# dblanm/gnn-manip

Measured on AMD Instinct MI355X. Metric: rollout steps/sec (N particles, 10 MP steps, hidden=128), higher is better.
Workload: dtype f32; 1 GPU; north_star target: N=100k dense synthetic scene, conn_r=0.015, max_neighbours=20, hidden=128, 10 MP steps; n_particles=100000, hidden=128, edges_last_step=1966056, k_steps=6, candidates_per_gpu=1, parallelism=candidate-parallel x1

## Files before the change

gnn_manip_amd/csrc/hedge.h:

```cpp
#pragma once
#include "common.h"
#include "mlp.h"

namespace gm {

struct EdgeBlockHeader {
    int n_blocks;
    int n_groups;
    int n_graphs;
    int n_per_graph;
    int n_stitch;
    int pad[3];
};
struct EdgeBlocks {
    EdgeBlockHeader* hdr;
    int* gblk;
    int2* blk;
    int2* seg;
    int* head;
    int* stitch;
    int* stitch_list;
    int64_t max_blocks;
};
size_t edge_blocks_ints(int64_t n_nodes, int64_t edge_capacity);
// ... 4 lines not shown

constexpr int kPackH3Max = 16;
struct PackH3Job {
    const float* W1;
    int W1_col0;
    int W1_ld;
    const float* W2;
    const float* W3;
    const float* b1;
    const float* b2;
    const float* b3;
    const float* gamma;
    const float* beta;
    float* dst;
    int enc_k1;
};
size_t h3_image_floats();
int pack_h3(const PackH3Job* jobs, int n, hipStream_t s);

int launch_edge_sys(const EdgeArgs& a, const EdgeBlocks& t, int64_t edge_capacity, hipStream_t s);
inline const float* edge_sys_p_scale(const float* h3_image) { return h3_image; }

struct NodeSysArgs {
    const float* h;
    const float* agg;
    const float* Q;
    float* h_out;
    const float* image;
    int n;
    int* flags;
// ... 5 lines not shown
struct ProjSysArgs {
    const float* h;
    float* P;
    float* Q;
    const float* img_p;
    const float* img_q;
    const float* scale_p;
    const float* scale_q;
    int n;
    int* flags;
    ProfState* prof;
    int precision;
};
int launch_proj_sys(const ProjSysArgs& a, hipStream_t s);
int launch_node_proj_sys(const NodeSysArgs& a, const ProjSysArgs& p, hipStream_t s);
int launch_agg_stitch(float* agg, const float* side, const EdgeBlocks& t, int64_t n, ProfState* prof, hipStream_t s);
constexpr int64_t kSysNodeMinNodes = 32 * 256 * 6;
int launch_edge_sys_enc(const EdgeArgs& a, hipStream_t s);
bool edge_sys_fits(int64_t n_nodes, int64_t edge_capacity);
constexpr int kEdgePadRows = 32;
int zero_edge_pad_rows(const CsrHeader* hdr, float* e, int row_floats, hipStream_t s);

}
```

gnn_manip_amd/csrc/hedge.hip:

```cpp
#include <type_traits>
#include "common.h"
#include "mlp.h"
#include "hedge.h"
#include "hmlp.h"
#include "hmma_dev.h"
#include "blocks_dev.h"

namespace gm {

namespace {

constexpr int H = 128;
constexpr int BE = 32;
constexpr int SYS_THREADS = 768;
static_assert(BE == kBlockEdges, "block tables and the systolic kernels agree on the block size");
#ifdef HEDGE_STAMPS
__device__ unsigned long long g_sys_stamps[3 * 32 * 8 + 32];
#define SYS_STAMP(tick, slot)                                                                                         \
    do {                                                                                                              \
        if (blockIdx.x == 0 && jb == 0 && lane0 == 0 && (tick) >= 16 && (tick) < 48) {                                \
            g_sys_stamps[(role * 32 + (tick) - 16) * 8 + (slot)] = __builtin_readcyclecounter();                     \
            if (role == 0 && (slot) == 0) g_sys_stamps[3 * 32 * 8 + (tick) - 16] = __builtin_amdgcn_s_memrealtime(); \
        }                                                                                                             \
    } while (0)
// ... 45 lines not shown
    return (g & 7) == 0 ? (i & 7) * (g >> 3) + (i >> 3) : i;
}

__device__ __forceinline__ int s_clamp0(int v, int hi) {
    int r;
    asm("s_max_i32 %0, %1, 0\n\ts_min_i32 %0, %0, %2" : "=s"(r) : "s"(v), "s"(hi) : "scc");
    return r;
}

extern __shared__ __attribute__((aligned(16))) char smem[];
#define LDS(T, off) (*reinterpret_cast<T*>(smem + (off)))
__device__ __forceinline__ unsigned opaque(unsigned v) { asm volatile("" : "+v"(v)); return v; }
__device__ __forceinline__ int tick_no(int t) { asm volatile("" : "+s"(t)); return t; }
#define GM_SB __builtin_amdgcn_sched_barrier(0)

template <int NP>
__device__ __forceinline__ void acc_to_image(const floatx16& a, char* smem, unsigned addr) {
#pragma unroll
    for (int q = 0; q < 2; ++q) {
        float v[8];
#pragma unroll
        for (int j = 0; j < 8; ++j) v[j] = relu(a[8 * q + j]);
        uintx2 h0, l0, h1, l1;
        if constexpr (NP == 3) {
            split4(v[0], v[1], v[2], v[3], h0, l0);
            split4(v[4], v[5], v[6], v[7], h1, l1);
        } else {
            hi4(v[0], v[1], v[2], v[3], h0);
            hi4(v[4], v[5], v[6], v[7], h1);
        }
        LDS(uintx4, addr + (q * 2 + 0) * 1024) = uintx4{h0[0], h0[1], h1[0], h1[1]};
        if constexpr (NP == 3) LDS(uintx4, addr + (q * 2 + 1) * 1024) = uintx4{l0[0], l0[1], l1[0], l1[1]};
    }
}

template <int NP, class F>
__device__ __forceinline__ void mlp_layer(floatx16& acc, const floatx16& c0, const half8 (&wh)[8], const half8 (&wl)[8], char* smem, unsigned a0, unsigned a1, F&& side) {
// ... 979 lines not shown
}

constexpr size_t NODE_PROJ_LDS_BYTES = NODE_LDS_BYTES > PROJ_LDS_BYTES ? NODE_LDS_BYTES : PROJ_LDS_BYTES;
static_assert(NODE_PROJ_LDS_BYTES <= 160 * 1024, "LDS budget");

template <int NP>
__global__ void __launch_bounds__(SYS_THREADS, 1) sys_node_proj_kernel(const float* a_h, float* a_h_out, const float* __restrict__ a_agg, float* a_Q, const float* __restrict__ a_hw,
                                                                            float* __restrict__ a_P, const float* __restrict__ a_wp, const float* __restrict__ a_wq,
                                                                            const float* __restrict__ a_sp, const float* __restrict__ a_sq, int a_n, int* a_flags,
                                                                            float a_eps) {
    sys_node_body<NP>(a_h, a_agg, a_Q, a_h_out, a_hw, a_n, a_flags, a_eps);
    __builtin_amdgcn_s_setprio(0);
    sys_proj_body<LD_SC1, NP>(a_h_out, a_P, a_Q, a_wp, a_wq, a_sp, a_sq, a_n, a_flags);
}

__global__ void __launch_bounds__(256) agg_stitch_kernel(float* __restrict__ agg, const float* __restrict__ side, const int* __restrict__ stitch,
                                                          const int* __restrict__ stitch_list, const int* __restrict__ head,
                                                          const EdgeBlockHeader* __restrict__ tab, int n) {
    const int ng = tab->n_groups, ns = tab->n_stitch;
    const int c = threadIdx.x & 7;
    for (int k = (blockIdx.x * 256 + threadIdx.x) >> 3; k < ns; k += (gridDim.x * 256) >> 3) {
        const int v = stitch_list[k];
        if (v < 0 || v >= n) continue;
        const int g0 = stitch[v];
        if (g0 < 0 || g0 >= ng || head[g0] != v) continue;
        floatx4 a[4];
#pragma unroll
        for (int q = 0; q < 4; ++q) a[q] = *reinterpret_cast<floatx4*>(agg + (size_t)v * H + 16 * c + 4 * q);
        int g = g0;
        do {
// ... 8 lines not shown

struct PackH3Jobs {
    int n;
    const float* W1[kPackH3Max];
    int c1[kPackH3Max];
    const float* W2[kPackH3Max];
    const float* W3[kPackH3Max];
    const float* b1[kPackH3Max];
    const float* b2[kPackH3Max];
    const float* b3[kPackH3Max];
    const float* gamma[kPackH3Max];
    const float* beta[kPackH3Max];
    float* dst[kPackH3Max];
    int enc_k1[kPackH3Max];
    int ld1[kPackH3Max];
};

constexpr int H3_PACK_THREADS = 1024;
__global__ void __launch_bounds__(H3_PACK_THREADS) pack_h3_kernel(PackH3Jobs J) {
    __shared__ float red[H3_PACK_THREADS];
    __shared__ float tsc[4];
    __shared__ float cmean[H + 1];
    const int job = blockIdx.x, tid = threadIdx.x;
    const float* Wl[3] = {J.W1[job], J.W2[job], J.W3[job]};
    if (tid < H) {
        float a = 0.f;
        for (int o = 0; o < H; ++o) a += J.W3[job][(size_t)o * H + tid];
        cmean[tid] = a * (1.0f / H);
    } else if (tid == H) {
        float a = 0.f;
        for (int o = 0; o < H; ++o) a += J.b3[job][o];
        cmean[H] = a * (1.0f / H);
    }
    __syncthreads();
    const int k1 = J.enc_k1[job];
    const bool enc = k1 > 0;
    const int ld[3] = {enc ? k1 : (J.ld1[job] > 0 ? J.ld1[job] : 3 * H), H, H}, c0[3] = {J.c1[job], 0, 0};
    const float* bl[3] = {J.b1[job], J.b2[job], J.b3[job]};
    float m_est = enc ? kHmRawInputRms : 1.f, U_prev = 1.f;
    if (tid == 0) tsc[3] = 0.f;
    __shared__ float capv;
    if (tid == 0) capv = 3.0e38f;
    for (int l = 0; l < 3; ++l) {
        float ss = 0.f, wm = 0.f;
        const int cols = l == 0 ? ld[0] : H;
        for (int i = tid; i < H * cols; i += H3_PACK_THREADS) {
            const int col = i % cols;
            float v = Wl[l][(size_t)(i / cols) * ld[l] + (l == 0 ? 0 : c0[l]) + col];
            if (l == 2) v -= cmean[col];
            ss = fmaf(v, v, ss);
            if (l != 0 || enc || (col >= c0[0] && col < c0[0] + H)) wm = fmaxf(wm, fabsf(v));
        }
        red[tid] = ss;
        __syncthreads();
        for (int s = H3_PACK_THREADS / 2; s > 0; s >>= 1) {
            if (tid < s) red[tid] += red[tid + s];
            __syncthreads();
        }
        const float ss_all = red[0];
        __syncthreads();
        red[tid] = wm;
        __syncthreads();
        for (int s = H3_PACK_THREADS / 2; s > 0; s >>= 1) {
            if (tid < s) red[tid] = fmaxf(red[tid], red[tid + s]);
            __syncthreads();
        }
        if (tid == 0) {
            const float wmax = red[0];
            float bs = 0.f, bmax = 0.f;
            for (int o = 0; o < H; ++o) {
                const float bv = bl[l][o] - (l == 2 ? cmean[H] : 0.f);
                bs = fmaf(bv, bv, bs);
                bmax = fmaxf(bmax, fabsf(bv));
            }
            const float g2 = ss_all / (float)H * 0.5f;
            float m = sqrtf(fmaf(enc ? 0.f : 0.5f, bs / (float)H, g2 * m_est * m_est));
            if (!(m > 1.0e-30f) || !(m < 1.0e30f)) m = 1.f;
            auto pow2 = [](float want, bool nearest) {
                if (!(want > 0.f) || !(want < 3.0e38f)) return 1.f;
                int ex;
                const float f = frexpf(want, &ex);
                int sh = (nearest && f >= 0.70710678f) ? ex : ex - 1;
                sh = sh < -100 ? -100 : (sh > 100 ? 100 : sh);
                return ldexpf(1.f, sh);
            };
            float t = pow2(kHmTargetRms / m, true) / U_prev;
            if (wmax > 0.f && wmax < 3.0e38f) {
                if (wmax * t > 8192.0f) t = pow2(8192.0f / wmax, false);
                if (wmax * t < 0.0625f) t = 2.f * pow2(0.0625f / wmax, false);
            }
            tsc[l] = t;
            tsc[3] = m;
            if (enc && bmax > 0.f) capv = fminf(capv, pow2(4096.0f / (U_prev * t * bmax), false));
        }
        __syncthreads();
        m_est = tsc[3];
        U_prev *= tsc[l];
        __syncthreads();
    }
    const float T1 = tsc[0], T2 = T1 * tsc[1], T3 = T2 * tsc[2];
    float* dst = J.dst[job];
    if (tid == 0) { dst[0] = T1; dst[1] = 1.0f / T3; dst[2] = capv; dst[3] = 0.f; }
    float* vec = dst + HW_HEADER_FLOATS;
    for (int i = tid; i < H; i += H3_PACK_THREADS) {
        vec[4 * H + i] = J.b1[job][i] * T1;
        vec[i] = J.b2[job][i] * T2;
        vec[H + i] = (J.b3[job][i] - cmean[H]) * T3;
        vec[2 * H + i] = J.gamma[job][i];
        vec[3 * H + i] = J.beta[job][i];
    }
    _Float16* img = reinterpret_cast<_Float16*>(dst + HW_HEADER_FLOATS + HW_VEC_FLOATS);
    for (int idx = tid; idx < 3 * 4 * 8 * 64 * 8; idx += H3_PACK_THREADS) {
        const int j = idx & 7, lane = (idx >> 3) & 63, ks = (idx >> 9) & 7, w = (idx >> 12) & 3, l = idx >> 14;
        const int i = lane & 31, kg = lane >> 5;
        const int kcol = 16 * ks + 8 * (j >> 2) + 4 * kg + (j & 3);
        const bool pad = l == 0 && enc && kcol >= k1;
        const float v = pad ? 0.f : (Wl[l][(size_t)(32 * w + i) * ld[l] + c0[l] + kcol] - (l == 2 ? cmean[kcol] : 0.f)) * tsc[l];
        const _Float16 h = (_Float16)v;
        const _Float16 lo = (_Float16)(v - (float)h);
        const size_t base = ((((size_t)(l * 4 + w) * 8 + ks) * 2) * 64 + lane) * 8 + j;
        img[base] = h;
        img[base + 64 * 8] = lo;
    }
}

__global__ void __launch_bounds__(256) edge_blocks_plan_kernel(const int* __restrict__ in_ptr, int n_nodes, const int* n_per_dev, int n_per_host,
                                                               EdgeBlockHeader* tab, int* gblk, int max_graphs) {
    if (threadIdx.x == 0) edge_blocks_plan(in_ptr, n_nodes, n_per_dev, n_per_host, tab, gblk, max_graphs);
}

__global__ void __launch_bounds__(256) edge_blocks_fill_kernel(const int* __restrict__ in_ptr, const int* __restrict__ dst, int n_nodes,
// ... 5 lines not shown

}

size_t h3_image_floats() { return (size_t)HW_HEADER_FLOATS + HW_VEC_FLOATS + (size_t)HW_IMAGE_HALF8 * 4; }

int pack_h3(const PackH3Job* jobs, int n, hipStream_t s) {
    for (int off = 0; off < n; off += kPackH3Max) {
        PackH3Jobs J{};
        J.n = n - off < kPackH3Max ? n - off : kPackH3Max;
        for (int i = 0; i < J.n; ++i) {
            const PackH3Job& j = jobs[off + i];
            J.W1[i] = j.W1; J.c1[i] = j.W1_col0; J.W2[i] = j.W2; J.W3[i] = j.W3; J.b1[i] = j.b1; J.b2[i] = j.b2; J.b3[i] = j.b3; J.gamma[i] = j.gamma; J.beta[i] = j.beta;
            J.dst[i] = j.dst;
            J.enc_k1[i] = j.enc_k1;
            J.ld1[i] = j.W1_ld;
        }
        hipLaunchKernelGGL(pack_h3_kernel, dim3(J.n), dim3(H3_PACK_THREADS), 0, s, J);
        GM_LAUNCH_CHECK();
    }
    return GM_OK;
}

static size_t max_blocks_of(int64_t n_nodes, int64_t edge_capacity) {
    return (size_t)cdiv(edge_capacity, BE) + 4 * (size_t)n_nodes + 4;
}
size_t edge_groups_max(int64_t n_nodes, int64_t edge_capacity) { return max_blocks_of(n_nodes, edge_capacity) / 4 + 1 + kSinkRows; }

size_t edge_blocks_ints(int64_t n_nodes, int64_t edge_capacity) {
    const size_t nblk = max_blocks_of(n_nodes, edge_capacity);
    return 8 + ((size_t)n_nodes + 2) + 1 + 4 * nblk + (nblk / 4 + 2) + 2 * (size_t)n_nodes;
// ... 97 lines not shown
}

int launch_node_proj_sys(const NodeSysArgs& a, const ProjSysArgs& p, hipStream_t s) {
    GM_REQUIRE(a.h && a.agg && a.Q && a.h_out && a.image && a.n > 0, GM_ERR_INVALID_ARGUMENT, "launch_node_proj_sys: bad argument");
    GM_REQUIRE(p.P && p.img_p && p.img_q, GM_ERR_INVALID_ARGUMENT, "launch_node_proj_sys: bad argument");
    GM_REQUIRE(p.h == a.h_out && p.Q == a.Q && p.n == a.n && p.flags == a.flags, GM_ERR_INVALID_ARGUMENT,
               "launch_node_proj_sys: the projection must read the node MLP's h_out and write its Q, over the same rows");
    GM_REQUIRE(p.precision == a.precision, GM_ERR_INVALID_ARGUMENT, "launch_node_proj_sys: the two halves disagree on the precision");
    auto go = [&](auto kern) {
        return launch_sys<decltype(kern)::value>(NODE_PROJ_LDS_BYTES, a.prof, PROF_NODE, s, a.h, a.h_out, a.agg, p.Q, a.image, p.P, p.img_p, p.img_q,
                                                 p.scale_p, p.scale_q, a.n, a.flags, a.eps);
    };
    return a.precision == kPrecisionF16 ? go(kernel_c<sys_node_proj_kernel<NP_F16>>{}) : go(kernel_c<sys_node_proj_kernel<NP_F32>>{});
}

int launch_agg_stitch(float* agg, const float* side, const EdgeBlocks& t, int64_t n, ProfState* prof_state, hipStream_t s) {
    if (n <= 0) return GM_OK;
    {
        ProfScope prof(prof_state, PROF_NODE, s);
        int64_t gb = cdiv(n * 8, 256 * 4);
        gb = gb < 1 ? 1 : (gb > 2048 ? 2048 : gb);
        hipLaunchKernelGGL(agg_stitch_kernel, dim3((unsigned)gb), dim3(256), 0, s, agg, side, t.stitch, t.stitch_list, t.head, t.hdr, (int)n);
    }
    GM_LAUNCH_CHECK();
    return GM_OK;
}

__global__ void __launch_bounds__(256) edge_pad_rows_kernel(const CsrHeader* hdr, float* e, int row_floats) {
    const size_t base = (size_t)hdr->n_edges * row_floats;
    for (int i = blockIdx.x * blockDim.x + threadIdx.x; i < kEdgePadRows * row_floats; i += gridDim.x * blockDim.x) e[base + i] = 0.f;
// ... 15 lines not shown
```

gnn_manip_amd/csrc/model.h:

```cpp
#pragma once
#include <mutex>
#include <vector>
#include "common.h"
#include "hmlp.h"
#include "mlp.h"
#include "train.h"

namespace gm {
enum EdgeKernel : int {
    EK_AUTO = 0,
    EK_SYS = 5,
    EK_HM = 6,
    EK_SYS_ALL = 7,
};

struct MlpSpec { int base, end, in, out; bool normed; };
struct TStream { size_t off = 0; int stages = 0, stages_tail = 0; };
std::vector<MlpSpec> model_mlps(const gm_model_desc& d);

inline int node_feature_dim(const gm_feature_desc* fd) { return 3 * (fd->k_steps - 1) + 7 + (fd->control_col >= 0 ? 3 : 0); }
inline int64_t graph_nodes(const gm_feature_desc* fd, int64_t n) { return fd->nodes_per_graph > 0 ? fd->nodes_per_graph : n; }
}

struct gm_model {
// ... 11 lines not shown
    std::vector<gm::VecJob> vec_jobs;
    size_t v_enc_edge, v_enc_node, v_dec;
    std::vector<size_t> v_edge, v_node;
    float* packed_t3 = nullptr;
    std::vector<gm::PackTJob> t_jobs;
    gm::TStream t_enc_edge, t_enc_node, t_dec;
    std::vector<gm::TStream> t_edge, t_node, t_proj;
    float* packed_hm = nullptr;
    std::vector<gm::PackHmJob> hm_jobs;
    gm::PackHmJob* hm_jobs_dev = nullptr;
    float* hm_stats = nullptr;
    size_t hm_enc_edge = 0, hm_enc_node = 0, hm_enc_node_tail = 0;
    std::vector<size_t> hm_edge, hm_node, hm_node_tail, hm_node_q;
    float* packed_h3 = nullptr;
    std::vector<gm::PackH3Job> h3_jobs;
    size_t h3_enc = 0;
    std::vector<size_t> h3_edge, h3_node;
    bool infer_stale = true;
    std::mutex lazy_mu;
    gm::ProfState* prof = nullptr;
    int edge_kernel = gm::EK_AUTO;
    bool node_fusion = true;
    int precision = gm::kPrecisionF32;
    hipEvent_t ready = nullptr;
    hipStream_t ready_stream = nullptr;
};
int ensure_inference_images(const gm_model* m, hipStream_t s);
int weights_ready_on(const gm_model* m, hipStream_t s);
```

gnn_manip_amd/csrc/model.hip:

```cpp
#include <algorithm>
#include <vector>
#include "common.h"
#include "mlp.h"
#include "model.h"
#include "train.h"
#include "hedge.h"
#include "hmlp.h"

using namespace gm;

std::vector<MlpSpec> gm::model_mlps(const gm_model_desc& d) {
    const int H = d.hidden_size, NL = d.num_layers;
    std::vector<MlpSpec> mlp;
    auto add = [&](int in, int out, bool normed) {
        const int base = mlp.empty() ? 0 : mlp.back().end;
        mlp.push_back({base, base + 2 * (NL + 1) + (normed ? 2 : 0), in, out, normed});
    };
    add(d.edge_dim, H, true);
    add(d.node_dim, H, true);
    for (int k = 0; k < d.m_steps; ++k) {
        add(3 * H, H, true);
        add(2 * H, H, true);
    }
    add(H, d.out_dim, false);
// ... 170 lines not shown
        if (k + 1 < M) proj(k + 1);
        else {
            head(1.f);
            for (int l = 0; l < NL; ++l) hh(dec.base + 2 * l);
            lin(dec.base + 2 * NL, Hv, 0, 0, dec.out, 32, 32, Hv, H, H, true, dec.out);
        }
    }
    for (int k = 0; k < M; ++k) {
        m->hm_node_q[k] = z.hm;
        head(1.f);
        lin(m->node_mlp(k).base, 2 * Hv, m->ch * Hv, 0, Hv, H, H, Hv, H, H, true, Hv);
    }

    m->h3_jobs.clear();
    if (Hv == 128 && NL == 2) {
        auto h3 = [&](size_t& slot, const MlpSpec& p, int W1_col0, int W1_ld, int enc_k1) {
            const float* const* W = &T[p.base];
            PackH3Job j{};
            j.W1 = W[0]; j.b1 = W[1]; j.W2 = W[2]; j.b2 = W[3]; j.W3 = W[4]; j.b3 = W[5]; j.gamma = W[6]; j.beta = W[7];
            j.W1_col0 = W1_col0; j.W1_ld = W1_ld; j.enc_k1 = enc_k1; j.dst = m->packed_h3 + z.h3;
            m->h3_jobs.push_back(j);
            slot = z.h3;
            z.h3 += h3_image_floats();
        };
        for (int k = 0; k < M; ++k) h3(m->h3_edge[k], m->edge_mlp(k), m->ce * H, 0, 0);
        h3(m->h3_enc, enc_edge, 0, 0, enc_edge.in);
        for (int k = 0; k < M; ++k) h3(m->h3_node[k], m->node_mlp(k), m->ca * H, 2 * H, 0);
    }
    return z;
}

template <class Batch, class Job>
int launch_batches(const std::vector<Job>& jobs, int (*launch)(const Batch&, float*, hipStream_t), float* base, hipStream_t s) {
    Batch b;
    const size_t cap = sizeof(b.job) / sizeof(b.job[0]);
    for (size_t i = 0; i < jobs.size(); i += cap) {
        b.n = (int)std::min(cap, jobs.size() - i);
        std::copy_n(jobs.begin() + i, b.n, b.job);
        const int rc = launch(b, base, s);
        if (rc != GM_OK) return rc;
    }
    return GM_OK;
}

int pack_common(const gm_model* m, hipStream_t s) {
    int rc = launch_batches(m->vec_jobs, launch_vec_batch, m->vec, s);
    if (rc == GM_OK && m->packed_t3) rc = launch_batches(m->t_jobs, launch_pack_b3_batch, m->packed_t3, s);
    return rc;
}

int pack_inference(const gm_model* m, hipStream_t s) {
    int rc = pack_hm(m->hm_jobs.data(), (int)m->hm_jobs.size(), m->hm_jobs_dev, m->hm_stats, s);
    if (rc != GM_OK || !m->packed_h3) return rc;
    const int n_edge = m->M + 1;
    rc = pack_h3(m->h3_jobs.data(), n_edge, s);
    if (rc == GM_OK) rc = pack_h3(m->h3_jobs.data() + n_edge, m->M, s);
    return rc;
}

int mark_ready(gm_model* m, hipStream_t s) {
    if (!m->ready) GM_HIP_CHECK(hipEventCreateWithFlags(&m->ready, hipEventDisableTiming));
    GM_HIP_CHECK(hipEventRecord(m->ready, s));
    m->ready_stream = s;
    return GM_OK;
}

int load_weights(gm_model* m, const float* const* T, int nt, bool on_device, hipStream_t s) {
    GM_REQUIRE(nt == (int)m->raw_jobs.size(), GM_ERR_INVALID_ARGUMENT, "model: expected %zu tensors, got %d", m->raw_jobs.size(), nt);
    for (int i = 0; i < nt; ++i) GM_REQUIRE(T[i] != nullptr, GM_ERR_INVALID_ARGUMENT, "model: tensor %d is null", i);
    std::lock_guard<std::mutex> guard(m->lazy_mu);
    int rc = GM_OK;
// ... 224 lines not shown
    if (cap > 0 && !route.sys_enc) {
        ProfScope prof(m->prof, PROF_REST, s);
        rc = zero_edge_pad_rows(c.hdr, f.e, H, s);
        if (rc != GM_OK) return rc;
    }
    auto proj_args = [&](int k) {
        ProjSysArgs pa{};
        pa.h = f.h; pa.P = f.P; pa.Q = f.Q; pa.n = (int)n; pa.flags = flags; pa.prof = m->prof;
        pa.precision = m->precision;
        pa.img_p = m->packed_hm + (k == 0 ? m->hm_enc_node_tail : m->hm_node_tail[k - 1]);
        pa.img_q = m->packed_hm + m->hm_node_q[k];
        pa.scale_p = edge_sys_p_scale(m->packed_h3 + m->h3_edge[k]);
        pa.scale_q = edge_sys_p_scale(m->packed_h3 + m->h3_node[k]);
        return pa;
    };
    {
        HmNodeArgs na = enc_node_args(m, n, nodes, f.h, flags);
        if (!route.sys_node) set_tail(m, na, 0, f.P, out, route.sys_edge);
        rc = launch_node_hm(H, 0, na, s);
    }
    if (rc == GM_OK && route.sys_node) rc = launch_proj_sys(proj_args(0), s);
    if (rc != GM_OK) return rc;
    if (!agg_cleared) {
        ProfScope prof(m->prof, PROF_REST, s);
        GM_HIP_CHECK(hipMemsetAsync(f.agg, 0, (size_t)n * H * sizeof(float), s));
    }
    for (int k = 0; k < M; ++k) {
        EdgeArgs ea = proc_edge_args(m, k, c, n, nullptr, f.P, f.e, f.e, f.agg, f.side, 1);
        ea.discard_e_out = k + 1 == M;
        ea.P_prescaled = route.sys_edge;
        rc = launch_edge(H, NL, false, route.sys_edge, ea, cap, s);
        if (rc != GM_OK) return rc;
        if (route.sys_node) {
            rc = launch_agg_stitch(f.agg, f.side, carve_edge_blocks(c.blocks, n, cap), n, m->prof, s);
            NodeSysArgs ns{};
            ns.h = f.h; ns.agg = f.agg; ns.Q = f.Q; ns.h_out = f.h; ns.image = m->packed_h3 + m->h3_node[k];
            ns.n = (int)n; ns.flags = flags; ns.eps = m->d.ln_eps; ns.prof = m->prof;
            ns.precision = m->precision;
            const bool fused = k + 1 < M && m->node_fusion;
            if (rc == GM_OK) rc = fused ? launch_node_proj_sys(ns, proj_args(k + 1), s) : launch_node_sys(ns, s);
            if (rc == GM_OK && k + 1 < M && !fused) rc = launch_proj_sys(proj_args(k + 1), s);
            if (rc == GM_OK && k + 1 == M) rc = launch_node_hm(H, 2, tail_args(m, M, n, f.h, f.P, out, flags), s);
        } else {
            HmNodeArgs a = proc_node_args(m, k, c, n, cap, f.h, f.agg, f.side, f.h, 1);
            set_tail(m, a, k + 1, f.P, out, route.sys_edge);
            rc = launch_node_hm(H, 1, a, s);
        }
        if (rc != GM_OK) return rc;
    }
    return GM_OK;
}
}

extern "C" {

int gm_epd_forward(const gm_model* m, const float* nodes, int64_t n, const float* edge_attr, int attr_is_csr_order,
                   const void* csr_ws, int64_t cap, float* out, void* fwd_ws, size_t fwd_ws_bytes, void* stream) {
// ... 263 lines not shown
```

Measured before the change: 129.0 rollout steps/s.

## Add systolic node-encoder and decoder kernels fused with projection and final node MLP

Adds a three-stage systolic kernel for the node encoder (with LayerNorm) that can be fused with the first P/Q projection. It also adds a systolic decoder kernel that can be fused with the last processor node MLP, replacing the generic launch_node_hm paths for encoder and tail when the systolic node route is active. Weight packing is extended with h3 images for the encoder and decoder, including a dec_out field and optional gamma/beta. The aim is to remove launches and intermediate h round-trips at the start and end of each forward pass, at the cost of much more kernel code and of new LDS layouts.

```diff
diff --git a/gnn_manip_amd/csrc/hedge.h b/gnn_manip_amd/csrc/hedge.h
--- a/gnn_manip_amd/csrc/hedge.h
+++ b/gnn_manip_amd/csrc/hedge.h
@@ -42,6 +42,7 @@
     const float* beta;
     float* dst;
     int enc_k1;
+    int dec_out;
 };
 size_t h3_image_floats();
 int pack_h3(const PackH3Job* jobs, int n, hipStream_t s);
@@ -77,6 +78,31 @@
 };
 int launch_proj_sys(const ProjSysArgs& a, hipStream_t s);
 int launch_node_proj_sys(const NodeSysArgs& a, const ProjSysArgs& p, hipStream_t s);
+struct NodeEncSysArgs {
+    const float* x;
+    int k1;
+    float* h_out;
+    const float* image;
+    int n;
+    int* flags;
+    float eps;
+    ProfState* prof;
+    int precision;
+};
+int launch_nenc_sys(const NodeEncSysArgs& a, hipStream_t s);
+int launch_nenc_proj_sys(const NodeEncSysArgs& a, const ProjSysArgs& p, hipStream_t s);
+struct DecSysArgs {
+    const float* h;
+    float* out;
+    int out_dim;
+    const float* image;
+    int n;
+    int* flags;
+    ProfState* prof;
+    int precision;
+};
+int launch_dec_sys(const DecSysArgs& a, hipStream_t s);
+int launch_node_dec_sys(const NodeSysArgs& a, const DecSysArgs& d, bool fused, hipStream_t s);
 int launch_agg_stitch(float* agg, const float* side, const EdgeBlocks& t, int64_t n, ProfState* prof, hipStream_t s);
 constexpr int64_t kSysNodeMinNodes = 32 * 256 * 6;
 int launch_edge_sys_enc(const EdgeArgs& a, hipStream_t s);
diff --git a/gnn_manip_amd/csrc/hedge.hip b/gnn_manip_amd/csrc/hedge.hip
--- a/gnn_manip_amd/csrc/hedge.hip
+++ b/gnn_manip_amd/csrc/hedge.hip
@@ -83,13 +83,14 @@
 __device__ __forceinline__ int tick_no(int t) { asm volatile("" : "+s"(t)); return t; }
 #define GM_SB __builtin_amdgcn_sched_barrier(0)
 
-template <int NP>
+template <int NP, bool POISON = false>
 __device__ __forceinline__ void acc_to_image(const floatx16& a, char* smem, unsigned addr) {
+    const float pois = POISON ? a[0] - a[0] : 0.f;
 #pragma unroll
     for (int q = 0; q < 2; ++q) {
         float v[8];
 #pragma unroll
-        for (int j = 0; j < 8; ++j) v[j] = relu(a[8 * q + j]);
+        for (int j = 0; j < 8; ++j) v[j] = POISON ? relu(a[8 * q + j]) + pois : relu(a[8 * q + j]);
         uintx2 h0, l0, h1, l1;
         if constexpr (NP == 3) {
             split4(v[0], v[1], v[2], v[3], h0, l0);
@@ -1099,6 +1100,339 @@
     sys_proj_body<LD_SC1, NP>(a_h_out, a_P, a_Q, a_wp, a_wq, a_sp, a_sq, a_n, a_flags);
 }
 
+#define NENC_TICKS(tick_as)                                                                          \
+    {                                                                                                \
+        auto tick = [&](auto par_c, int t) { tick_as(par_c, int_c<TICK_FULL>{}, t); };               \
+        RUN_TICKS(0, nb, tick);                                                                      \
+        if (nb & 1) {                                                                                \
+            tick(int_c<0>{}, nb + 1);                                                                \
+            tick_as(int_c<1>{}, int_c<TICK_DRAIN>{}, nb + 2);                                        \
+        } else {                                                                                     \
+            tick_as(int_c<0>{}, int_c<TICK_DRAIN>{}, nb + 2);                                        \
+        }                                                                                            \
+    }
+constexpr unsigned V_OOB = 0x40000000u;
+
+template <int NP>
+__device__ __forceinline__ void sys_nenc_body(const float* __restrict__ a_x, int a_k1, float* a_h_out, const float* __restrict__ a_hw, int a_n,
+                                              int* a_flags, float a_eps) {
+    const int tid = threadIdx.x, lane0 = tid & 63;
+    const int wave = __builtin_amdgcn_readfirstlane(tid >> 6);
+    const int role = wave >> 2, jb = wave & 3;
+    const int N = a_n;
+    const int nblk = (N + BE - 1) / BE;
+    const int2 br = wg_range(nblk, false);
+    const int b0 = br.x, b1 = br.y;
+    const int nb = b1 - b0;
+    if (nb <= 0) return;
+    const float inv_T = a_hw[1], cap = a_hw[2];
+    half8 wh[8], wl[8];
+    sys_prologue<NP>(wh, wl, reinterpret_cast<const half8*>(a_hw + HW_HEADER_FLOATS + HW_VEC_FLOATS), role * 4 + jb, false, LE_ZERO_END, LE_VEC,
+                     a_hw + HW_HEADER_FLOATS, 5 * H);
+    const int n = lane0 & 31, hi = lane0 >> 5, rr = lane0 >> 3, cq = lane0 & 7;
+    const int r0 = b0 * BE;
+    const int rows_wg = (b1 * BE < N ? b1 * BE : N) - r0;
+    const floatx16 bv = vec_to_acc(smem, LE_VEC, (role == 0 ? 4 : role - 1) * H, jb, hi);
+    const unsigned rs_l = opaque(LE_RS + n * 4);
+    int rng = 0;
+    floatx16 acc;
+    auto scaled_bias = [&](float sc) {
+        floatx16 c;
+#pragma unroll
+        for (int r = 0; r < 16; ++r) c[r] = bv[r] * sc;
+        return c;
+    };
+    set_role_prio(role);
+    if (role == 0) {
+        const unsigned row_b = (unsigned)a_k1 * 4u;
+        const srd_t srd_x = make_srd(a_x + (size_t)r0 * a_k1, (unsigned)(rows_wg > 0 ? rows_wg : 0) * row_b);
+        const int f_part = a_k1 & ~3, n_part = a_k1 & 3;
+        const int q_part = f_part >> 3;
+        const bool mine = n_part != 0 && ((f_part >> 2) & 1) == hi;
+        unsigned v_xq[4], v_xp[3];
+#pragma unroll
+        for (int q = 0; q < 4; ++q) v_xq[q] = opaque(8 * q + 4 * hi + 4 <= a_k1 ? n * row_b + (8 * q + 4 * hi) * 4u : V_OOB);
+#pragma unroll
+        for (int i = 0; i < 3; ++i) v_xp[i] = opaque(mine && i < n_part ? n * row_b + (f_part + i) * 4u : V_OOB);
+        float* const h_out_wg = a_h_out + (size_t)r0 * H;
+        const unsigned v_eoff = opaque(rr * 512 + jb * 128 + cq * 16);
+        const unsigned x1_w = opaque(LE_X1 + 4 * jb * 1024 + lane0 * 16);
+        const unsigned st_r = opaque(LE_ST + n * 4);
+        const unsigned km_w = opaque(LE_KM + jb * 128 + n * 4), km_r = opaque(LE_KM + jb * 128 + rr * 4);
+        const unsigned z_r = opaque(LE_Z + jb * TILE_B + rr * TILE_ROW_B + cq * 16);
+        const floatx4 gm = LDS(floatx4, LE_VEC + (2 * H + 32 * jb + 4 * cq) * 4);
+        const floatx4 bt = LDS(floatx4, LE_VEC + (3 * H + 32 * jb + 4 * cq) * 4);
+        const float T3 = 1.0f / inv_T;
+        floatx4 xq[4];
+        float xp[3];
+        auto request = [&](unsigned soff) {
+#pragma unroll
+            for (int q = 0; q < 4; ++q) xq[q] = bld4(srd_x, v_xq[q], soff);
+#pragma unroll
+            for (int i = 0; i < 3; ++i) xp[i] = __uint_as_float(__builtin_amdgcn_raw_buffer_load_b32(srd_x, v_xp[i], soff, 0));
+        };
+        request(0);
+        auto tick_as = [&](auto par_c, auto kind_c, int t) {
+            constexpr int PAR = decltype(par_c)::value, P3 = 1 - PAR, KIND = decltype(kind_c)::value;
+            const int x = b0 + t;
+            if constexpr (KIND == TICK_FULL) {
+                float mx = 0.f;
+#pragma unroll
+                for (int q = 0; q < 4; ++q) {
+                    const bool here = mine && q == q_part;
+#pragma unroll
+                    for (int i = 0; i < 4; ++i) {
+                        if (here) xq[q][i] = i < 3 ? xp[i] : 0.f;
+                        mx = fmaxf(mx, fabsf(xq[q][i]));
+                    }
+                }
+                {
+                    const auto r = __builtin_amdgcn_permlane32_swap(__float_as_uint(mx), __float_as_uint(mx), false, false);
+                    mx = fmaxf(__uint_as_float(r[0]), __uint_as_float(r[1]));
+                }
+                float sc = cap;
+                if (mx > 0.f && mx < 3.0e38f) {
+                    int ex;
+                    (void)frexpf(mx, &ex);
+                    sc = fminf(ldexpf(1.f, min(7 - ex, 100)), cap);
+                }
+                if (jb == 0 && hi == 0) LDS(float, rs_l + (x & (RS_SLOTS - 1)) * 128) = sc;
+                uintx2 h[4], l[4];
+#pragma unroll
+                for (int q = 0; q < 4; ++q) {
+                    if constexpr (NP == 3) split4(xq[q][0] * sc, xq[q][1] * sc, xq[q][2] * sc, xq[q][3] * sc, h[q], l[q]);
+                    else hi4(xq[q][0] * sc, xq[q][1] * sc, xq[q][2] * sc, xq[q][3] * sc, h[q]);
+                }
+                const floatx16 c0v = scaled_bias(sc);
+                request((unsigned)((x + 1 < b1 ? x + 1 : b1 - 1) - b0) * (BE * row_b));
+#pragma unroll
+                for (int ks = 0; ks < 2; ++ks) {
+                    const half8 bh = __builtin_bit_cast(half8, uintx4{h[2 * ks][0], h[2 * ks][1], h[2 * ks + 1][0], h[2 * ks + 1][1]});
+                    if constexpr (NP == 3) {
+                        const half8 bl = __builtin_bit_cast(half8, uintx4{l[2 * ks][0], l[2 * ks][1], l[2 * ks + 1][0], l[2 * ks + 1][1]});
+                        acc = __builtin_amdgcn_mfma_f32_32x32x16_f16(wl[ks], bh, ks == 0 ? c0v : acc, 0, 0, 0);
+                        acc = __builtin_amdgcn_mfma_f32_32x32x16_f16(wh[ks], bl, acc, 0, 0, 0);
+                        acc = __builtin_amdgcn_mfma_f32_32x32x16_f16(wh[ks], bh, acc, 0, 0, 0);
+                    } else {
+                        acc = __builtin_amdgcn_mfma_f32_32x32x16_f16(wh[ks], bh, ks == 0 ? c0v : acc, 0, 0, 0);
+                    }
+                }
+            }
+            {
+                const float rs3 = LDS(float, rs_l + ((x - 3) & (RS_SLOTS - 1)) * 128);
+                const float q = (LDS(float, st_r + P3 * 512) + LDS(float, st_r + P3 * 512 + 128)) + (LDS(float, st_r + P3 * 512 + 256) + LDS(float, st_r + P3 * 512 + 384));
+                const float tt3 = T3 * rs3;
+                const float v = fmaf(a_eps * tt3, tt3, q * (1.0f / 128.0f));
+                float r = __builtin_amdgcn_rsqf(v);
+                r = r * fmaf(-0.5f * v * r, r, 1.5f);
+                LDS(float, km_w) = r;
+                const int xb = x - 3;
+                const int cnt = (xb >= b0 && xb < b1) ? min(BE, N - xb * BE) : 0;
+#pragma unroll
+                for (int j = 0; j < 4; ++j) {
+                    const float kr = LDS(float, km_r + j * 32);
+                    const floatx4 zq = LDS(floatx4, z_r + P3 * 4 * TILE_B + j * 8 * TILE_ROW_B);
+                    floatx4 o;
+#pragma unroll
+                    for (int tt = 0; tt < 4; ++tt) o[tt] = fmaf(zq[tt] * kr, gm[tt], bt[tt]);
+                    bst4(make_srd(h_out_wg + (size_t)((xb < b0 ? 0 : xb - b0) * BE + 8 * j) * H, (unsigned)s_clamp0(cnt - 8 * j, 8) * 512u), v_eoff, 0, o);
+                }
+            }
+            if constexpr (KIND == TICK_FULL) {
+                rng |= __any(row_bad<NP>(acc[0])) ? 1 : 0;
+                GM_SB;
+                acc_to_image<NP, true>(acc, smem, x1_w + PAR * IMG_B);
+            }
+            lds_barrier();
+        };
+        NENC_TICKS(tick_as);
+    } else if (role == 1) {
+        const unsigned x_in = opaque(LE_X1 + lane0 * 16), x_out = opaque(LE_X2 + 4 * jb * 1024 + lane0 * 16);
+        auto nothing = [](int) {};
+        auto tick_as = [&](auto par_c, auto kind_c, int t) {
+            constexpr int PAR = decltype(par_c)::value, P1 = 1 - PAR, KIND = decltype(kind_c)::value;
+            if constexpr (KIND == TICK_FULL) {
+                const int x = b0 + t;
+                const floatx16 c0v = scaled_bias(LDS(float, rs_l + ((x - 1) & (RS_SLOTS - 1)) * 128));
+                mlp_layer<NP>(acc, c0v, wh, wl, smem, x_in + P1 * IMG_B, x_in + P1 * IMG_B, nothing);
+                rng |= __any(row_bad<NP>(acc[0])) ? 1 : 0;
+                GM_SB;
+                acc_to_image<NP, true>(acc, smem, x_out + P1 * IMG_B);
+            }
+            lds_barrier();
+        };
+        NENC_TICKS(tick_as);
+    } else {
+        const unsigned x_in = opaque(LE_X2 + lane0 * 16);
+        const unsigned st_w = opaque(LE_ST + jb * 128 + n * 4);
+        const unsigned z_w = opaque(LE_Z + jb * TILE_B + n * TILE_ROW_B + hi * 16);
+        auto nothing = [](int) {};
+        auto tick_as = [&](auto par_c, auto kind_c, int t) {
+            constexpr int PAR = decltype(par_c)::value, P2 = PAR, KIND = decltype(kind_c)::value;
+            if constexpr (KIND == TICK_FULL) {
+                const int x = b0 + t;
+                const floatx16 c0v = scaled_bias(LDS(float, rs_l + ((x - 2) & (RS_SLOTS - 1)) * 128));
+                mlp_layer<NP>(acc, c0v, wh, wl, smem, x_in + P2 * IMG_B, x_in + P2 * IMG_B, nothing);
+                rng |= __any(row_bad<NP>(acc[0])) ? 1 : 0;
+                publish_ln_stats(acc, st_w + P2 * 512, z_w + P2 * 4 * TILE_B);
+            }
+            lds_barrier();
+        };
+        NENC_TICKS(tick_as);
+    }
+    report_split_range(rng, lane0, a_flags);
+}
+
+template <int NP>
+__global__ void __launch_bounds__(SYS_THREADS, 1) sys_nenc_kernel(const float* __restrict__ a_x, int a_k1, float* a_h_out, const float* __restrict__ a_hw, int a_n,
+                                                                       int* a_flags, float a_eps) {
+    sys_nenc_body<NP>(a_x, a_k1, a_h_out, a_hw, a_n, a_flags, a_eps);
+}
+
+template <int NP>
+__global__ void __launch_bounds__(SYS_THREADS, 1) sys_nenc_proj_kernel(const float* __restrict__ a_x, int a_k1, float* a_h_out, const float* __restrict__ a_hw,
+                                                                            float* __restrict__ a_P, float* __restrict__ a_Q, const float* __restrict__ a_wp,
+                                                                            const float* __restrict__ a_wq, const float* __restrict__ a_sp,
+                                                                            const float* __restrict__ a_sq, int a_n, int* a_flags, float a_eps) {
+    sys_nenc_body<NP>(a_x, a_k1, a_h_out, a_hw, a_n, a_flags, a_eps);
+    __builtin_amdgcn_s_setprio(0);
+    sys_proj_body<LD_SC1, NP>(a_h_out, a_P, a_Q, a_wp, a_wq, a_sp, a_sq, a_n, a_flags);
+}
+constexpr size_t NENC_PROJ_LDS_BYTES = ENC_LDS_BYTES > PROJ_LDS_BYTES ? ENC_LDS_BYTES : PROJ_LDS_BYTES;
+static_assert(NENC_PROJ_LDS_BYTES <= 160 * 1024, "LDS budget");
+
+constexpr int LDEC_E = 0;
+constexpr int LDEC_X1 = LDEC_E + 2 * IMG_B;
+constexpr int LDEC_X2 = LDEC_X1 + 2 * IMG_B;
+constexpr int LDEC_ZERO_END = LDEC_X2 + 2 * IMG_B;
+constexpr int LDEC_VEC = LDEC_ZERO_END;
+constexpr size_t DEC_LDS_BYTES = LDEC_VEC + 5 * H * 4;
+
+template <int LD_H, int NP>
+__device__ __forceinline__ void sys_dec_body(const float* __restrict__ a_h, float* __restrict__ a_out, const float* __restrict__ a_hw, int a_n,
+                                             int a_out_dim, int* a_flags) {
+    const int tid = threadIdx.x, lane0 = tid & 63;
+    const int wave = __builtin_amdgcn_readfirstlane(tid >> 6);
+    const int role = wave >> 2, jb = wave & 3;
+    const int N = a_n;
+    const int nblk = (N + BE - 1) / BE;
+    const int2 br = wg_range(nblk, false);
+    const int b0 = br.x, b1 = br.y;
+    const int nb = b1 - b0;
+    if (nb <= 0) return;
+    const bool poisoned = a_flags && (*reinterpret_cast<volatile int*>(a_flags) & ERRF_SPLIT_RANGE) != 0;
+    const float inv_T = a_hw[1];
+    half8 wh[8], wl[8];
+    sys_prologue<NP>(wh, wl, reinterpret_cast<const half8*>(a_hw + HW_HEADER_FLOATS + HW_VEC_FLOATS), role * 4 + jb, false, LDEC_ZERO_END, LDEC_VEC,
+                     a_hw + HW_HEADER_FLOATS, 5 * H);
+    const int n = lane0 & 31, hi = lane0 >> 5, rr = lane0 >> 3, cq = lane0 & 7;
+    const int r0 = b0 * BE;
+    const int rows_wg = (b1 * BE < N ? b1 * BE : N) - r0;
+    const unsigned wg_bytes = (unsigned)(rows_wg > 0 ? rows_wg : 0) * 512u;
+    const floatx16 bv = vec_to_acc(smem, LDEC_VEC, (role == 0 ? 4 : role - 1) * H, jb, hi);
+    auto clampb = [&](int x) { return x < b0 ? b0 : (x < b1 ? x : b1 - 1); };
+    int rng = 0;
+    floatx16 acc;
+    set_role_prio(role);
+    if (role == 0) {
+        const srd_t srd_h = make_srd(a_h + (size_t)r0 * H, wg_bytes);
+        const unsigned v_eoff = opaque(rr * 512 + jb * 128 + cq * 16);
+        const int kg = cq & 1, ksb = cq >> 2, half = (cq >> 1) & 1;
+        const unsigned e_w = opaque(LDEC_E + ((2 * jb + ksb) * 2 * 64 + ((rr ^ (2 * (ksb + 2 * kg))) + 32 * kg)) * 16 + half * 8);
+        const unsigned e_r0 = opaque(LDEC_E + eslot(n, hi, 0) * 16), e_r1 = opaque(LDEC_E + eslot(n, hi, 1) * 16);
+        const unsigned x1_w = opaque(LDEC_X1 + 4 * jb * 1024 + lane0 * 16);
+        floatx4 eq[4];
+#pragma unroll
+        for (int j = 0; j < 4; ++j) eq[j] = bld4s<LD_H>(srd_h, v_eoff, j * 4096);
+        auto tick_as = [&](auto par_c, auto kind_c, int t) {
+            constexpr int PAR = decltype(par_c)::value, KIND = decltype(kind_c)::value;
+            const int x = b0 + t;
+            const unsigned rel2 = (unsigned)(clampb(x + 2) - b0) * (BE * 512u);
+            auto side = [&](int slot) {
+                if (slot < 8 && !(slot & 1)) {
+                    const int j = slot >> 1;
+                    uintx2 h, l;
+                    if constexpr (NP == 3) split4(eq[j][0], eq[j][1], eq[j][2], eq[j][3], h, l);
+                    else hi4(eq[j][0], eq[j][1], eq[j][2], eq[j][3], h);
+                    LDS(uintx2, e_w + (1 - PAR) * IMG_B + j * 128) = h;
+                    if constexpr (NP == 3) LDS(uintx2, e_w + (1 - PAR) * IMG_B + j * 128 + 1024) = l;
+                } else if (slot == 8) {
+#pragma unroll
+                    for (int j = 0; j < 4; ++j) eq[j] = bld4s<LD_H>(srd_h, v_eoff, rel2 + j * 4096);
+                }
+            };
+            if constexpr (KIND == TICK_FULL) {
+                mlp_layer<NP>(acc, bv, wh, wl, smem, e_r0 + PAR * IMG_B, e_r1 + PAR * IMG_B, side);
+                rng |= __any(row_bad<NP>(acc[0])) ? 1 : 0;
+                GM_SB;
+                acc_to_image<NP, true>(acc, smem, x1_w + PAR * IMG_B);
+            } else {
+#pragma unroll
+                for (int slot = 0; slot <= 8; ++slot) side(slot);
+            }
+            lds_barrier();
+        };
+        auto tick = [&](auto par_c, int t) { tick_as(par_c, int_c<TICK_FULL>{}, t); };
+        tick_as(int_c<1>{}, int_c<TICK_FILL>{}, -1);
+        RUN_TICKS(0, nb, tick);
+        if (nb & 1) tick(int_c<0>{}, nb + 1);
+    } else if (role == 1) {
+        const unsigned x_in = opaque(LDEC_X1 + lane0 * 16), x_out = opaque(LDEC_X2 + 4 * jb * 1024 + lane0 * 16);
+        auto nothing = [](int) {};
+        auto tick = [&](auto par_c, int) {
+            constexpr int PIN = 1 - decltype(par_c)::value;
+            mlp_layer<NP>(acc, bv, wh, wl, smem, x_in + PIN * IMG_B, x_in + PIN * IMG_B, nothing);
+            rng |= __any(row_bad<NP>(acc[0])) ? 1 : 0;
+            GM_SB;
+            acc_to_image<NP, true>(acc, smem, x_out + PIN * IMG_B);
+            lds_barrier();
+        };
+        lds_barrier();
+        RUN_TICKS(0, nb, tick);
+        if (nb & 1) tick(int_c<0>{}, nb + 1);
+    } else if (jb != 0) {
+        for (int t = -1; t <= nb + 1; ++t) lds_barrier();
+    } else {
+        const unsigned x_in = opaque(LDEC_X2 + lane0 * 16);
+        unsigned v_out[4];
+#pragma unroll
+        for (int tt = 0; tt < 4; ++tt) v_out[tt] = opaque(4 * hi + tt < a_out_dim ? (unsigned)(n * a_out_dim + 4 * hi + tt) * 4u : V_OOB);
+        float* const out_wg = a_out + (size_t)r0 * a_out_dim;
+        auto nothing = [](int) {};
+        auto tick = [&](auto par_c, int t) {
+            constexpr int PAR = decltype(par_c)::value;
+            const int xb = b0 + t - 2;
+            mlp_layer<NP>(acc, bv, wh, wl, smem, x_in + PAR * IMG_B, x_in + PAR * IMG_B, nothing);
+            rng |= __any(row_bad<NP>(acc[0])) ? 1 : 0;
+            const int cnt = (xb >= b0 && xb < b1) ? min(BE, N - xb * BE) : 0;
+            const srd_t srd_o = make_srd(out_wg + (size_t)((xb < b0 ? 0 : xb - b0) * BE) * a_out_dim, (unsigned)(cnt * a_out_dim) * 4u);
+            const bool bad = poisoned || rng;
+#pragma unroll
+            for (int tt = 0; tt < 4; ++tt) bst1s<0>(srd_o, v_out[tt], 0, bad ? __builtin_nanf("") : acc[tt] * inv_T);
+            lds_barrier();
+        };
+        lds_barrier();
+        RUN_TICKS(0, nb, tick);
+        if (nb & 1) tick(int_c<0>{}, nb + 1);
+    }
+    report_split_range(rng, lane0, a_flags);
+}
+
+template <int NP>
+__global__ void __launch_bounds__(SYS_THREADS, 1) sys_dec_kernel(const float* __restrict__ a_h, float* __restrict__ a_out, const float* __restrict__ a_hw, int a_n,
+                                                                      int a_out_dim, int* a_flags) {
+    sys_dec_body<0, NP>(a_h, a_out, a_hw, a_n, a_out_dim, a_flags);
+}
+
+template <int NP>
+__global__ void __launch_bounds__(SYS_THREADS, 1) sys_node_dec_kernel(const float* a_h, float* a_h_out, const float* __restrict__ a_agg, const float* __restrict__ a_Q,
+                                                                           const float* __restrict__ a_hw, float* __restrict__ a_out, const float* __restrict__ a_hw_dec,
+                                                                           int a_n, int a_out_dim, int* a_flags, float a_eps) {
+    sys_node_body<NP>(a_h, a_agg, a_Q, a_h_out, a_hw, a_n, a_flags, a_eps);
+    sys_dec_body<LD_SC1, NP>(a_h_out, a_out, a_hw_dec, a_n, a_out_dim, a_flags);
+}
+constexpr size_t NODE_DEC_LDS_BYTES = NODE_LDS_BYTES > DEC_LDS_BYTES ? NODE_LDS_BYTES : DEC_LDS_BYTES;
+
 __global__ void __launch_bounds__(256) agg_stitch_kernel(float* __restrict__ agg, const float* __restrict__ side, const int* __restrict__ stitch,
                                                           const int* __restrict__ stitch_list, const int* __restrict__ head,
                                                           const EdgeBlockHeader* __restrict__ tab, int n) {
@@ -1137,6 +1471,7 @@
     float* dst[kPackH3Max];
     int enc_k1[kPackH3Max];
     int ld1[kPackH3Max];
+    int dec_out[kPackH3Max];
 };
 
 constexpr int H3_PACK_THREADS = 1024;
@@ -1146,13 +1481,15 @@
     __shared__ float cmean[H + 1];
     const int job = blockIdx.x, tid = threadIdx.x;
     const float* Wl[3] = {J.W1[job], J.W2[job], J.W3[job]};
+    const bool dec = J.dec_out[job] > 0;
+    const int out3 = dec ? J.dec_out[job] : H;
     if (tid < H) {
         float a = 0.f;
-        for (int o = 0; o < H; ++o) a += J.W3[job][(size_t)o * H + tid];
+        for (int o = 0; o < H && !dec; ++o) a += J.W3[job][(size_t)o * H + tid];
         cmean[tid] = a * (1.0f / H);
     } else if (tid == H) {
         float a = 0.f;
-        for (int o = 0; o < H; ++o) a += J.b3[job][o];
+        for (int o = 0; o < H && !dec; ++o) a += J.b3[job][o];
         cmean[H] = a * (1.0f / H);
     }
     __syncthreads();
@@ -1167,7 +1504,8 @@
     for (int l = 0; l < 3; ++l) {
         float ss = 0.f, wm = 0.f;
         const int cols = l == 0 ? ld[0] : H;
-        for (int i = tid; i < H * cols; i += H3_PACK_THREADS) {
+        const int outs = l == 2 ? out3 : H;
+        for (int i = tid; i < outs * cols; i += H3_PACK_THREADS) {
             const int col = i % cols;
             float v = Wl[l][(size_t)(i / cols) * ld[l] + (l == 0 ? 0 : c0[l]) + col];
             if (l == 2) v -= cmean[col];
@@ -1191,13 +1529,13 @@
         if (tid == 0) {
             const float wmax = red[0];
             float bs = 0.f, bmax = 0.f;
-            for (int o = 0; o < H; ++o) {
+            for (int o = 0; o < outs; ++o) {
                 const float bv = bl[l][o] - (l == 2 ? cmean[H] : 0.f);
                 bs = fmaf(bv, bv, bs);
                 bmax = fmaxf(bmax, fabsf(bv));
             }
-            const float g2 = ss_all / (float)H * 0.5f;
-            float m = sqrtf(fmaf(enc ? 0.f : 0.5f, bs / (float)H, g2 * m_est * m_est));
+            const float g2 = ss_all / (float)outs * 0.5f;
+            float m = sqrtf(fmaf(enc ? 0.f : 0.5f, bs / (float)outs, g2 * m_est * m_est));
             if (!(m > 1.0e-30f) || !(m < 1.0e30f)) m = 1.f;
             auto pow2 = [](float want, bool nearest) {
                 if (!(want > 0.f) || !(want < 3.0e38f)) return 1.f;
@@ -1228,16 +1566,16 @@
     for (int i = tid; i < H; i += H3_PACK_THREADS) {
         vec[4 * H + i] = J.b1[job][i] * T1;
         vec[i] = J.b2[job][i] * T2;
-        vec[H + i] = (J.b3[job][i] - cmean[H]) * T3;
-        vec[2 * H + i] = J.gamma[job][i];
-        vec[3 * H + i] = J.beta[job][i];
+        vec[H + i] = i < out3 ? (J.b3[job][i] - cmean[H]) * T3 : 0.f;
+        vec[2 * H + i] = dec ? 0.f : J.gamma[job][i];
+        vec[3 * H + i] = dec ? 0.f : J.beta[job][i];
     }
     _Float16* img = reinterpret_cast<_Float16*>(dst + HW_HEADER_FLOATS + HW_VEC_FLOATS);
     for (int idx = tid; idx < 3 * 4 * 8 * 64 * 8; idx += H3_PACK_THREADS) {
         const int j = idx & 7, lane = (idx >> 3) & 63, ks = (idx >> 9) & 7, w = (idx >> 12) & 3, l = idx >> 14;
         const int i = lane & 31, kg = lane >> 5;
         const int kcol = 16 * ks + 8 * (j >> 2) + 4 * kg + (j & 3);
-        const bool pad = l == 0 && enc && kcol >= k1;
+        const bool pad = (l == 0 && enc && kcol >= k1) || (l == 2 && 32 * w + i >= out3);
         const float v = pad ? 0.f : (Wl[l][(size_t)(32 * w + i) * ld[l] + c0[l] + kcol] - (l == 2 ? cmean[kcol] : 0.f)) * tsc[l];
         const _Float16 h = (_Float16)v;
         const _Float16 lo = (_Float16)(v - (float)h);
@@ -1273,6 +1611,7 @@
             J.dst[i] = j.dst;
             J.enc_k1[i] = j.enc_k1;
             J.ld1[i] = j.W1_ld;
+            J.dec_out[i] = j.dec_out;
         }
         hipLaunchKernelGGL(pack_h3_kernel, dim3(J.n), dim3(H3_PACK_THREADS), 0, s, J);
         GM_LAUNCH_CHECK();
@@ -1400,6 +1739,61 @@
     return a.precision == kPrecisionF16 ? go(kernel_c<sys_node_proj_kernel<NP_F16>>{}) : go(kernel_c<sys_node_proj_kernel<NP_F32>>{});
 }
 
+int launch_nenc_sys(const NodeEncSysArgs& a, hipStream_t s) {
+    GM_REQUIRE(a.x && a.h_out && a.image && a.n > 0 && a.k1 >= 1 && a.k1 <= 32, GM_ERR_INVALID_ARGUMENT, "launch_nenc_sys: bad argument");
+    auto go = [&](auto kern) {
+        return launch_sys<decltype(kern)::value>(ENC_LDS_BYTES, a.prof, PROF_ENC, s, a.x, a.k1, a.h_out, a.image, a.n, a.flags, a.eps);
+    };
+    return a.precision == kPrecisionF16 ? go(kernel_c<sys_nenc_kernel<NP_F16>>{}) : go(kernel_c<sys_nenc_kernel<NP_F32>>{});
+}
+
+int launch_nenc_proj_sys(const NodeEncSysArgs& a, const ProjSysArgs& p, hipStream_t s) {
+    GM_REQUIRE(a.x && a.h_out && a.image && a.n > 0 && a.k1 >= 1 && a.k1 <= 32, GM_ERR_INVALID_ARGUMENT, "launch_nenc_proj_sys: bad argument");
+    GM_REQUIRE(p.P && p.Q && p.img_p && p.img_q, GM_ERR_INVALID_ARGUMENT, "launch_nenc_proj_sys: bad argument");
+    GM_REQUIRE(p.h == a.h_out && p.n == a.n && p.flags == a.flags && p.precision == a.precision, GM_ERR_INVALID_ARGUMENT,
+               "launch_nenc_proj_sys: the projection must read the encoder's h_out, over the same rows and at its precision");
+    auto go = [&](auto kern) {
+        return launch_sys<decltype(kern)::value>(NENC_PROJ_LDS_BYTES, a.prof, PROF_NODE, s, a.x, a.k1, a.h_out, a.image, p.P, p.Q, p.img_p, p.img_q,
+                                                 p.scale_p, p.scale_q, a.n, a.flags, a.eps);
+    };
+    return a.precision == kPrecisionF16 ? go(kernel_c<sys_nenc_proj_kernel<NP_F16>>{}) : go(kernel_c<sys_nenc_proj_kernel<NP_F32>>{});
+}
+
+static int check_dec_args(const DecSysArgs& a, const char* who) {
+    GM_REQUIRE(a.h && a.out && a.image && a.n > 0 && a.out_dim >= 1 && a.out_dim <= 8, GM_ERR_INVALID_ARGUMENT, "%s: bad argument", who);
+    GM_REQUIRE((uint64_t)a.n * a.out_dim * 4 < (1ull << 31), GM_ERR_INVALID_ARGUMENT, "%s: output too large", who);
+    return GM_OK;
+}
+
+int launch_dec_sys(const DecSysArgs& a, hipStream_t s) {
+    const int rc = check_dec_args(a, "launch_dec_sys");
+    if (rc != GM_OK) return rc;
+    auto go = [&](auto kern) { return launch_sys<decltype(kern)::value>(DEC_LDS_BYTES, a.prof, PROF_NODE, s, a.h, a.out, a.image, a.n, a.out_dim, a.flags); };
+    return a.precision == kPrecisionF16 ? go(kernel_c<sys_dec_kernel<NP_F16>>{}) : go(kernel_c<sys_dec_kernel<NP_F32>>{});
+}
+
+int launch_node_dec_sys(const NodeSysArgs& a, const DecSysArgs& d, bool fused, hipStream_t s) {
+    GM_REQUIRE(a.h && a.agg && a.Q && a.h_out && a.image && a.n > 0, GM_ERR_INVALID_ARGUMENT, "launch_node_dec_sys: bad argument");
+    const int rc = check_dec_args(d, "launch_node_dec_sys");
+    if (rc != GM_OK) return rc;
+    GM_REQUIRE(d.h == a.h_out && d.n == a.n && d.flags == a.flags && d.precision == a.precision, GM_ERR_INVALID_ARGUMENT,
+               "launch_node_dec_sys: the decoder must read the node MLP's h_out, over the same rows and at its precision");
+    if (!fused) {
+        ProfScope prof(a.prof, PROF_NODE, s);
+        NodeSysArgs a1 = a;
+        DecSysArgs d1 = d;
+        a1.prof = nullptr;
+        d1.prof = nullptr;
+        const int rc_node = launch_node_sys(a1, s);
+        return rc_node != GM_OK ? rc_node : launch_dec_sys(d1, s);
+    }
+    auto go = [&](auto kern) {
+        return launch_sys<decltype(kern)::value>(NODE_DEC_LDS_BYTES, a.prof, PROF_NODE, s, a.h, a.h_out, a.agg, a.Q, a.image, d.out, d.image, a.n, d.out_dim,
+                                                 a.flags, a.eps);
+    };
+    return a.precision == kPrecisionF16 ? go(kernel_c<sys_node_dec_kernel<NP_F16>>{}) : go(kernel_c<sys_node_dec_kernel<NP_F32>>{});
+}
+
 int launch_agg_stitch(float* agg, const float* side, const EdgeBlocks& t, int64_t n, ProfState* prof_state, hipStream_t s) {
     if (n <= 0) return GM_OK;
     {
diff --git a/gnn_manip_amd/csrc/model.h b/gnn_manip_amd/csrc/model.h
--- a/gnn_manip_amd/csrc/model.h
+++ b/gnn_manip_amd/csrc/model.h
@@ -49,7 +49,7 @@
     std::vector<size_t> hm_edge, hm_node, hm_node_tail, hm_node_q;
     float* packed_h3 = nullptr;
     std::vector<gm::PackH3Job> h3_jobs;
-    size_t h3_enc = 0;
+    size_t h3_enc = 0, h3_nenc = 0, h3_dec = 0;
     std::vector<size_t> h3_edge, h3_node;
     bool infer_stale = true;
     std::mutex lazy_mu;
diff --git a/gnn_manip_amd/csrc/model.hip b/gnn_manip_amd/csrc/model.hip
--- a/gnn_manip_amd/csrc/model.hip
+++ b/gnn_manip_amd/csrc/model.hip
@@ -208,11 +208,12 @@
 
     m->h3_jobs.clear();
     if (Hv == 128 && NL == 2) {
-        auto h3 = [&](size_t& slot, const MlpSpec& p, int W1_col0, int W1_ld, int enc_k1) {
+        auto h3 = [&](size_t& slot, const MlpSpec& p, int W1_col0, int W1_ld, int enc_k1, int dec_out = 0) {
             const float* const* W = &T[p.base];
             PackH3Job j{};
-            j.W1 = W[0]; j.b1 = W[1]; j.W2 = W[2]; j.b2 = W[3]; j.W3 = W[4]; j.b3 = W[5]; j.gamma = W[6]; j.beta = W[7];
-            j.W1_col0 = W1_col0; j.W1_ld = W1_ld; j.enc_k1 = enc_k1; j.dst = m->packed_h3 + z.h3;
+            j.W1 = W[0]; j.b1 = W[1]; j.W2 = W[2]; j.b2 = W[3]; j.W3 = W[4]; j.b3 = W[5];
+            if (p.normed) { j.gamma = W[6]; j.beta = W[7]; }
+            j.W1_col0 = W1_col0; j.W1_ld = W1_ld; j.enc_k1 = enc_k1; j.dec_out = dec_out; j.dst = m->packed_h3 + z.h3;
             m->h3_jobs.push_back(j);
             slot = z.h3;
             z.h3 += h3_image_floats();
@@ -220,6 +221,8 @@
         for (int k = 0; k < M; ++k) h3(m->h3_edge[k], m->edge_mlp(k), m->ce * H, 0, 0);
         h3(m->h3_enc, enc_edge, 0, 0, enc_edge.in);
         for (int k = 0; k < M; ++k) h3(m->h3_node[k], m->node_mlp(k), m->ca * H, 2 * H, 0);
+        h3(m->h3_nenc, enc_node, 0, 0, enc_node.in);
+        h3(m->h3_dec, dec, 0, H, 0, dec.out);
     }
     return z;
 }
@@ -248,7 +251,7 @@
     if (rc != GM_OK || !m->packed_h3) return rc;
     const int n_edge = m->M + 1;
     rc = pack_h3(m->h3_jobs.data(), n_edge, s);
-    if (rc == GM_OK) rc = pack_h3(m->h3_jobs.data() + n_edge, m->M, s);
+    if (rc == GM_OK) rc = pack_h3(m->h3_jobs.data() + n_edge, (int)m->h3_jobs.size() - n_edge, s);
     return rc;
 }
 
@@ -503,12 +506,17 @@
         pa.scale_q = edge_sys_p_scale(m->packed_h3 + m->h3_node[k]);
         return pa;
     };
-    {
+    if (route.sys_node) {
+        NodeEncSysArgs ne{};
+        ne.x = nodes; ne.k1 = m->d.node_dim; ne.h_out = f.h; ne.image = m->packed_h3 + m->h3_nenc;
+        ne.n = (int)n; ne.flags = flags; ne.eps = m->d.ln_eps; ne.prof = m->prof; ne.precision = m->precision;
+        rc = m->node_fusion ? launch_nenc_proj_sys(ne, proj_args(0), s) : launch_nenc_sys(ne, s);
+        if (rc == GM_OK && !m->node_fusion) rc = launch_proj_sys(proj_args(0), s);
+    } else {
         HmNodeArgs na = enc_node_args(m, n, nodes, f.h, flags);
-        if (!route.sys_node) set_tail(m, na, 0, f.P, out, route.sys_edge);
+        set_tail(m, na, 0, f.P, out, route.sys_edge);
         rc = launch_node_hm(H, 0, na, s);
     }
-    if (rc == GM_OK && route.sys_node) rc = launch_proj_sys(proj_args(0), s);
     if (rc != GM_OK) return rc;
     if (!agg_cleared) {
         ProfScope prof(m->prof, PROF_REST, s);
@@ -526,10 +534,15 @@
             ns.h = f.h; ns.agg = f.agg; ns.Q = f.Q; ns.h_out = f.h; ns.image = m->packed_h3 + m->h3_node[k];
             ns.n = (int)n; ns.flags = flags; ns.eps = m->d.ln_eps; ns.prof = m->prof;
             ns.precision = m->precision;
-            const bool fused = k + 1 < M && m->node_fusion;
-            if (rc == GM_OK) rc = fused ? launch_node_proj_sys(ns, proj_args(k + 1), s) : launch_node_sys(ns, s);
-            if (rc == GM_OK && k + 1 < M && !fused) rc = launch_proj_sys(proj_args(k + 1), s);
-            if (rc == GM_OK && k + 1 == M) rc = launch_node_hm(H, 2, tail_args(m, M, n, f.h, f.P, out, flags), s);
+            if (rc == GM_OK && k + 1 < M) {
+                rc = m->node_fusion ? launch_node_proj_sys(ns, proj_args(k + 1), s) : launch_node_sys(ns, s);
+                if (rc == GM_OK && !m->node_fusion) rc = launch_proj_sys(proj_args(k + 1), s);
+            } else if (rc == GM_OK) {
+                DecSysArgs da{};
+                da.h = f.h; da.out = out; da.out_dim = m->d.out_dim; da.image = m->packed_h3 + m->h3_dec;
+                da.n = (int)n; da.flags = flags; da.prof = m->prof; da.precision = m->precision;
+                rc = launch_node_dec_sys(ns, da, m->node_fusion, s);
+            }
         } else {
             HmNodeArgs a = proc_node_args(m, k, c, n, cap, f.h, f.agg, f.side, f.h, 1);
             set_tail(m, a, k + 1, f.P, out, route.sys_edge);
```

Measured after the change: 129.4 rollout steps/s (median of 6 runs). Within noise of the previous version (+0.3%).
